# BUTSpeechFIT/VBx

Measured on NVIDIA H100. Metric: x-vectors/sec through 10 VB-HMM EM iters, higher is better.
Workload: dtype f32

## Files before the change

### include/vbx_b200.h

```cpp
#ifndef VBX_B200_H
#define VBX_B200_H

#include <stddef.h>
#include <stdint.h>

#ifdef __cplusplus
extern "C" {
#endif

typedef struct vbx_handle_s *vbx_handle_t;

enum vbx_status {
    VBX_OK = 0,
    VBX_ERR_ARG = -1,
    VBX_ERR_CUDA = -2,
    VBX_ERR_STATE = -3,
    VBX_ERR_NO_DEVICE = -4
};

enum vbx_flag {
    VBX_FLAG_NONFINITE = 1,
    VBX_FLAG_ELBO_DECREASED = 2,
    VBX_FLAG_CONVERGED = 4
};
// ... 134 lines not shown
int vbx_combine_workspace_bytes(vbx_handle_t h, int32_t n_rec, int32_t K, int32_t max_labels, size_t *bytes_out);
int vbx_combine(vbx_handle_t h, int32_t n_rec, const int64_t *offsets, int64_t N, const int64_t *lo, const int64_t *hi,
                int32_t K, const int32_t *labels, const int32_t *labels2, const int32_t *n_labels, int32_t max_labels,
                const double *weights, void *workspace, size_t workspace_bytes, int32_t *labels_out,
                int32_t *labels2_out, int32_t *order_out, double *weights_out, int64_t *D_out, int32_t *map_out,
                int32_t *n_global_out, int32_t *flags_out, int64_t *O_out, int64_t *L_out, void *stream);

int vbx_class_scatter_workspace_bytes(vbx_handle_t h, int64_t N, int32_t D, int32_t K, size_t *bytes_out);
int vbx_class_scatter(vbx_handle_t h, const float *X, int64_t N, int32_t D, int32_t K, const int64_t *offsets,
                      void *workspace, size_t workspace_bytes, double *means_out, double *scatter_out, void *stream);

int vbx_stream_window(vbx_handle_t h, int32_t n, int32_t C, int32_t R, int32_t S_max, int32_t S, const int32_t *slot,
                      const int64_t *blk_off, const int64_t *win_off, const int32_t *blk_lab, const int32_t *n_clusters,
                      const float *blk_fea, double smoothing, const float *ctx_fea, const int32_t *ctx_lab,
                      const int64_t *count, const int32_t *K, const double *n_hist, const double *F_hist, float *fea_out,
                      float *gamma_out, float *pi_out, int32_t *n_states_out, double *prior_n_out, double *prior_F_out,
                      void *stream);
int vbx_stream_commit(vbx_handle_t h, int32_t n, int32_t C, int32_t R, int32_t S_max, const int32_t *slot,
                      const int64_t *blk_off, const int64_t *win_off, const float *blk_fea, const int32_t *first,
                      float *ctx_fea, int32_t *ctx_lab, int64_t *count, int32_t *K, double *n_hist, double *F_hist,
                      int32_t *labels_out, void *stream);

int64_t vbx_launch_count(vbx_handle_t h);

enum vbx_kernel_class {
    VBX_K_PROJECT = 0,
    VBX_K_PREPARE = 1,
    VBX_K_RUN_INIT = 2,
    VBX_K_MSTEP = 3,
    VBX_K_SPEAKER_MODEL = 4,
    VBX_K_LOGLIK = 5,
    VBX_K_FWDBWD = 6,
    VBX_K_EXACT64 = 7,
    VBX_N_KERNEL_CLASSES = 8
};
int vbx_get_timings(vbx_handle_t h, double *ms_out, int64_t *count_out, int32_t reset);

#ifdef __cplusplus
}
#endif
#endif
```

### vbx_b200/_lib.py

```python
import ctypes
import os

_HERE = os.path.dirname(os.path.abspath(__file__))
LIB_PATH = os.environ.get('VBX_B200_LIB', os.path.join(_HERE, 'libvbx_b200.so'))

EXPORTS = ['vbx_version', 'vbx_padded_states', 'vbx_padded_states_wide', 'vbx_create', 'vbx_destroy', 'vbx_last_error',
           'vbx_set_option', 'vbx_plan', 'vbx_bind_workspace', 'vbx_prepare_scale',
           'vbx_prepare_project', 'vbx_prepare_xvectors', 'vbx_run', 'vbx_run_per_recording', 'vbx_hard_labels', 'vbx_hard_labels_keep', 'vbx_ahc_workspace_bytes', 'vbx_ahc', 'vbx_launch_count', 'vbx_get_timings', 'vbx_f64_workspace_bytes',
           'vbx_run_f64', 'vbx_plan_f64', 'vbx_forward_backward', 'vbx_attach_comm', 'vbx_elbo_trace', 'vbx_get_gsum',
           'vbx_score', 'vbx_score_overlap', 'vbx_score_jer', 'vbx_link_batch_workspace_bytes', 'vbx_link_batch',
           'vbx_enroll_batch_workspace_bytes', 'vbx_enroll_batch', 'vbx_cohort_stats_batch_workspace_bytes',
           'vbx_cohort_stats_batch', 'vbx_init_turns', 'vbx_combine_workspace_bytes', 'vbx_combine',
           'vbx_init_random', 'vbx_run_prior', 'vbx_run_f64_prior', 'vbx_class_scatter_workspace_bytes',
           'vbx_class_scatter', 'vbx_stream_window', 'vbx_stream_commit']

FLAG_NONFINITE, FLAG_ELBO_DECREASED, FLAG_CONVERGED = 1, 2, 4
SCORE_BAD_LABEL, SCORE_BAD_REGION, SCORE_BAD_RECORDING = 1, 2, 4
COMBINE_BAD_LABEL, COMBINE_TOO_MANY_LABELS = 1, 2
LINK_MAX_SPEAKERS = 1 << 29
KERNEL_CLASSES = ['project', 'prepare', 'run_init', 'mstep_partial', 'speaker_model', 'loglik', 'forward_backward', 'exact64']


class VbxError(RuntimeError):
    pass


_lib = None


def load():
    global _lib
    if _lib is not None:
        return _lib
    if not os.path.exists(LIB_PATH):
        raise VbxError(f'{LIB_PATH} is missing - run `python -c "import __graft_entry__ as g; g.build()"` '
                       '(there is no CPU fallback for the VB-HMM path)')
    lib = ctypes.CDLL(LIB_PATH)
    vp, i32, i64, dbl = ctypes.c_void_p, ctypes.c_int32, ctypes.c_int64, ctypes.c_double
    lib.vbx_version.restype = ctypes.c_char_p
    lib.vbx_version.argtypes = []
    lib.vbx_padded_states.restype = i32
    lib.vbx_padded_states.argtypes = [i32]
    lib.vbx_padded_states_wide.restype = i32
    lib.vbx_padded_states_wide.argtypes = [i32]
    lib.vbx_create.restype = ctypes.c_int
    lib.vbx_create.argtypes = [i32, ctypes.POINTER(vp)]
    lib.vbx_destroy.restype = ctypes.c_int
    lib.vbx_destroy.argtypes = [vp]
    lib.vbx_last_error.restype = ctypes.c_char_p
    lib.vbx_last_error.argtypes = [vp]
    lib.vbx_set_option.restype = ctypes.c_int
    lib.vbx_set_option.argtypes = [vp, ctypes.c_char_p, i32]
    lib.vbx_plan.restype = ctypes.c_int
# ... 98 lines not shown
```

### vbx_b200/build.py

```python
import os
import subprocess

HERE = os.path.dirname(os.path.abspath(__file__))
CSRC = os.path.join(HERE, 'csrc')
LIB = os.path.join(HERE, 'libvbx_b200.so')
SOURCES = ['vbx_kernels.cu', 'vbx_mma_kernels.cu', 'vbx_long_kernels.cu', 'vbx_fb_split.cu', 'vbx_project_tc.cu', 'vbx_f64.cu', 'vbx_exact64.cu', 'vbx_fb_dense.cu', 'vbx_ahc.cu',
           'vbx_score.cu', 'vbx_count.cu', 'vbx_link.cu', 'vbx_enroll.cu', 'vbx_cohort.cu', 'vbx_init.cu', 'vbx_combine.cu',
           'vbx_train.cu', 'vbx_stream.cu', 'vbx_capi.cu']
ARCH = ['-gencode', 'arch=compute_90a,code=sm_90a']
NVCC_FLAGS = ARCH + ['-lineinfo', '-O3', '-std=c++17', '-Xcompiler', '-fPIC', '-Xptxas', '-v']


def _nvcc():
    for cand in (os.environ.get('NVCC'), '/usr/local/cuda/bin/nvcc', 'nvcc'):
        if cand and (os.path.isabs(cand) and os.path.exists(cand) or not os.path.isabs(cand)):
            return cand
    raise RuntimeError('nvcc not found')


def needs_build():
    if not os.path.exists(LIB):
        return True
    t = os.path.getmtime(LIB)
    deps = [os.path.join(CSRC, f) for f in os.listdir(CSRC) if f.endswith(('.cu', '.cuh', '.h'))]
    deps += [os.path.join(HERE, '..', 'include', 'vbx_b200.h'), os.path.abspath(__file__)]
    return any(os.path.getmtime(d) > t for d in deps)


def build_library(force=False, verbose=False):
    if not force and not needs_build():
        return LIB
    nvcc = _nvcc()
    objs = []
    logs = []
    for src in SOURCES:
        obj = os.path.join(CSRC, src.replace('.cu', '.o'))
        cmd = [nvcc] + NVCC_FLAGS + ['-c', os.path.join(CSRC, src), '-o', obj]
        r = subprocess.run(cmd, capture_output=True, text=True)
        logs.append(r.stderr)
        if r.returncode != 0:
            raise RuntimeError('nvcc failed for %s:\n%s\n%s' % (src, r.stdout, r.stderr))
# ... 15 lines not shown
```

### vbx_b200/csrc/vbx_capi.cu

```cuda
#include <dlfcn.h>
#include <nvtx3/nvToolsExt.h>

#include <algorithm>
#include <cmath>
#include <cstdio>
#include <cstring>
#include <initializer_list>
#include <numeric>
#include <string>
#include <utility>
#include <vector>

#include "../../include/vbx_b200.h"
#include "vbx_internal.cuh"

struct vbx_handle_s {
    int device = 0;
    int sms = 0;
    std::string err;
    vbx::Plan plan;
    vbx::Workspace ws;
    bool planned = false, bound = false, prepared = false;
    bool f64_only = false;
    size_t ws_need = 0;
// ... 348 lines not shown
    if (h->plan_mem) {
        cudaFree(h->plan_mem);
        h->plan_mem = nullptr;
    }
    h->planned = h->bound = h->prepared = false;
    h->f64_only = false;
    drop_graph(h);
    e = cudaMalloc(&h->plan_mem, off);
    if (e != cudaSuccess) return cuda_fail(h, e, "cudaMalloc(plan)");
    char *base = static_cast<char *>(h->plan_mem);
    auto up = [&](size_t o, const void *src, size_t bytes) {
        return bytes ? cudaMemcpy(base + o, src, bytes, cudaMemcpyHostToDevice) : cudaSuccess;
    };
    if ((e = up(o_off, offsets_host, sizeof(int64_t) * (n_rec + 1))) != cudaSuccess ||
        (e = up(o_ord, order.data(), sizeof(int32_t) * n_rec)) != cudaSuccess ||
        (e = up(o_lrec, lrec.data(), sizeof(int32_t) * lrec.size())) != cudaSuccess ||
        (e = up(o_lf0, lf0.data(), sizeof(int64_t) * lf0.size())) != cudaSuccess ||
        (e = up(o_mrec, mrec.data(), sizeof(int32_t) * mrec.size())) != cudaSuccess ||
        (e = up(o_mf0, mf0.data(), sizeof(int64_t) * mf0.size())) != cudaSuccess ||
        (e = up(o_mb, mbegin.data(), sizeof(int32_t) * (n_rec + 1))) != cudaSuccess ||
        (e = up(o_ll, lrec_list.data(), sizeof(int32_t) * lrec_list.size())) != cudaSuccess ||
        (e = up(o_lf, lrec_first.data(), sizeof(int32_t) * lrec_first.size())) != cudaSuccess ||
        (e = up(o_ln, lrec_nchunks.data(), sizeof(int32_t) * lrec_nchunks.size())) != cudaSuccess ||
        (e = up(o_lcr, lchunk_rec.data(), sizeof(int32_t) * lchunk_rec.size())) != cudaSuccess ||
        (e = up(o_lci, lchunk_idx.data(), sizeof(int32_t) * lchunk_idx.size())) != cudaSuccess)
        return cuda_fail(h, e, "cudaMemcpy(plan)");

    vbx::Plan &pl = h->plan;
    pl.n_rec = n_rec;
    pl.R = R;
    pl.S = S;
    pl.exact = h->opt_exact_stop;
    pl.split = split ? 1 : 0;
    pl.n_frames = n_rec ? offsets_host[n_rec] : 0;
    pl.n_ltiles = (int32_t)lrec.size();
    pl.n_mtiles = (int32_t)mrec.size();
    pl.max_T = maxT;
    pl.offsets = reinterpret_cast<const int64_t *>(base + o_off);
    pl.order = reinterpret_cast<const int32_t *>(base + o_ord);
    pl.ltile_rec = reinterpret_cast<const int32_t *>(base + o_lrec);
    pl.ltile_f0 = reinterpret_cast<const int64_t *>(base + o_lf0);
    pl.mtile_rec = reinterpret_cast<const int32_t *>(base + o_mrec);
    pl.mtile_f0 = reinterpret_cast<const int64_t *>(base + o_mf0);
    pl.mtile_begin = reinterpret_cast<const int32_t *>(base + o_mb);
    pl.n_lrec = (int32_t)lrec_list.size();
    pl.n_lchunks = (int32_t)lchunk_rec.size();
    pl.lrec_list = reinterpret_cast<const int32_t *>(base + o_ll);
    pl.lrec_first = reinterpret_cast<const int32_t *>(base + o_lf);
    pl.lrec_nchunks = reinterpret_cast<const int32_t *>(base + o_ln);
    pl.lchunk_rec = reinterpret_cast<const int32_t *>(base + o_lcr);
    pl.lchunk_idx = reinterpret_cast<const int32_t *>(base + o_lci);
    h->ws_need = carve(pl, nullptr, nullptr);
    h->offsets_host.assign(offsets_host, offsets_host + (n_rec ? n_rec + 1 : 0));
    if (n_rec == 0) h->offsets_host.assign(1, 0);
    h->ahc_need = vbx::ahc_workspace_bytes(h->offsets_host.data(), n_rec, &h->ahc_d_off);
    h->planned = true;
    if (workspace_bytes_out) *workspace_bytes_out = h->ws_need;
    return VBX_OK;
}

int vbx_plan_f64(vbx_handle_t h, const int64_t *offsets_host, int32_t n_rec, int32_t R, int32_t S) {
    if (!h || !offsets_host || n_rec < 0) return fail(h, VBX_ERR_ARG, "vbx_plan_f64: null argument");
    if (R < 1 || S < 1 || S > 3600) return fail(h, VBX_ERR_ARG, "vbx_plan_f64: need R >= 1 and 1 <= S <= 3600");
    if (n_rec > 0 && offsets_host[0] != 0) return fail(h, VBX_ERR_ARG, "vbx_plan_f64: offsets[0] must be 0");
    for (int b = 0; b < n_rec; ++b) {
        const int64_t T = offsets_host[b + 1] - offsets_host[b];
// ... 181 lines not shown
    if (!per_rec && !(Fb != 0.0)) return fail(h, VBX_ERR_ARG, w + ": Fb must be non-zero");
    if (per_rec && (!Fa_v || !Fb_v || !loopP_v)) return fail(h, VBX_ERR_ARG, w + ": Fa, Fb and loop_prob must be device arrays [n_rec]");
    if (warm_start && (!alpha_io || !invL_io)) return fail(h, VBX_ERR_ARG, w + ": warm_start needs alpha_io and invL_io");
    const vbx::Plan &pl = h->plan;
    if (pl.n_rec == 0) return VBX_OK;
    if (!Li_out || !n_iters_out || !flags_out || !pi_io) return fail(h, VBX_ERR_ARG, w + ": null output pointer");
    if (pl.n_frames && (!rho || !Phi || !gamma_io)) return fail(h, VBX_ERR_ARG, w + ": null pointer");
    if ((rc = misaligned16(h, w, {{rho, "rho"}, {gamma_io, "gamma_io"}}))) return rc;
    vbx::RunParams rp;
    rp.epsilon = epsilon;
    rp.max_iters = max_iters;
    rp.hybrid = (pl.exact && epsilon > -1e300 && epsilon < 1e300 && max_iters > 1) ? 1 : 0;
    rp.warm = warm_start ? 1 : 0;

    auto enqueue = [&](cudaStream_t st) -> int {
    int rc = 0;
    {
        Timed t(h, st, VBX_K_RUN_INIT);
        rc = counted(h, vbx::launch_run_init(pl, h->ws, gamma_io, n_states, Li_out, n_iters_out, flags_out, max_iters, Fa, Fb,
                                             loop_prob, Fa_v, Fb_v, loopP_v, st), "run_init");
    }
    if (rc) return rc;
    const int rounds = max_iters + (rp.hybrid ? 1 : 0);
    const bool fb_hi = !pl.split && pl.n_rec >= 1024;
    for (int it = 0; it < rounds; ++it) {
        Range nvtx_iter("vbx_em_iteration");
        const bool given = it == 0 && warm_start;
        if (it < max_iters) {
            if (rp.hybrid) {
                Timed t(h, st, VBX_K_EXACT64);
                rc = counted(h, vbx::launch_snapshot(pl, h->ws, gamma_io, pi_io, it, st), "snapshot");
                if (rc) return rc;
            }
            if (!given) {
                Timed t(h, st, VBX_K_MSTEP);
                rc = counted(h, h->opt_gemm ? vbx::launch_mstep_partial(pl, h->ws, rho, gamma_io, st)
                                            : vbx::launch_mstep_mma(pl, h->ws, rho, gamma_io, st), "mstep_partial");
            }
            if (rc) return rc;
            {
                Timed t(h, st, VBX_K_SPEAKER_MODEL);
                rc = counted(h, vbx::launch_speaker_model(pl, h->ws, Phi, n_states, alpha_io, invL_io, given, st, prior_n,
                                                          prior_F), "speaker_model");
            }
            if (rc) return rc;
            {
                Timed t(h, st, VBX_K_LOGLIK);
                rc = counted(h, h->opt_gemm ? vbx::launch_loglik(pl, h->ws, rho, pi_io, n_states, st) : vbx::launch_loglik_mma(pl, h->ws, rho, pi_io, n_states, st), "loglik");
            }
            if (rc) return rc;
            if (fb_hi) {
                cudaEventRecord(h->ev_fork, st);
                cudaStreamWaitEvent(h->hi_stream, h->ev_fork, 0);
            }
            {
                cudaStream_t fs = fb_hi ? h->hi_stream : st;
                Timed t(h, fs, VBX_K_FWDBWD);
                rc = counted(h, vbx::launch_forward_backward(pl, h->ws, rp, gamma_io, pi_io, n_states, Li_out, n_iters_out, flags_out, it, h->opt_fb_spl, h->opt_fb_classic, h->opt_fb_ring, fs), "forward_backward");
            }
            if (fb_hi) {
                cudaEventRecord(h->ev_join, h->hi_stream);
                cudaStreamWaitEvent(st, h->ev_join, 0);
            }
            if (rc) return rc;
        }
        if (rp.hybrid && it > 0) {
            Timed t(h, st, VBX_K_EXACT64);
            rc = counted(h, vbx::launch_exact64_round(pl, h->ws, rp, rho, Phi, gamma_io, pi_io, n_states, alpha_io, invL_io, Li_out,
                                                      n_iters_out, flags_out, st, prior_n, prior_F), "exact64");
            if (rc) return rc;
        }
    }
    return VBX_OK;
    };

    cudaStream_t user = (cudaStream_t)stream;
    const bool want_graph = (h->opt_graph == 1 || (h->opt_graph == 0 && pl.split)) && !h->opt_timing && !h->opt_debug_sync &&
                            !h->graph_broken;
    if (!want_graph) return enqueue(user);
    uint64_t key = 1469598103934665603ull;
    auto mix = [&](uint64_t v) { key = (key ^ v) * 1099511628211ull; };
    auto bits = [](double d) { uint64_t u; memcpy(&u, &d, 8); return u; };
    for (const void *p : {(const void *)rho, (const void *)Phi, (const void *)gamma_io, (const void *)pi_io, (const void *)n_states,
// ... 727 lines not shown
```

### vbx_b200/csrc/vbx_internal.cuh

```cuda
#pragma once
#include <cuda_runtime.h>
#include <stdint.h>

#include <string>
#include <vector>

#define VBX_EPS_TR 1e-8f

namespace vbx {

constexpr int kLTile = 64;
constexpr int kMTile = 512;
constexpr int kLongT = 4096;
constexpr int kChunk = 256;
constexpr int kMaxR = 128;
constexpr int kMaxS = 64;
constexpr int kMaxSWide = 128;
constexpr int kTcMaxD = 2048;

struct Plan {
    int32_t n_rec = 0, R = 0, S = 0;
    int32_t exact = 0;
    int32_t split = 0;
    int64_t n_frames = 0;
    int32_t n_ltiles = 0, n_mtiles = 0;
    int64_t max_T = 0;
    const int64_t *offsets = nullptr;
    const int32_t *order = nullptr;
    const int32_t *ltile_rec = nullptr;
    const int64_t *ltile_f0 = nullptr;
    const int32_t *mtile_rec = nullptr;
    const int64_t *mtile_f0 = nullptr;
    const int32_t *mtile_begin = nullptr;
    int32_t n_lrec = 0, n_lchunks = 0;
    const int32_t *lrec_list = nullptr;
    const int32_t *lrec_first = nullptr;
    const int32_t *lrec_nchunks = nullptr;
    const int32_t *lchunk_rec = nullptr;
    const int32_t *lchunk_idx = nullptr;
};

struct RecParams {
    float Fa, Fb, FaFb, loopP;
    double dFa, dFb, dFaFb, dloopP;
};

struct Workspace {
    float *p = nullptr;
    float *rowmax = nullptr;
    float *rsigma = nullptr;
    float *cvec = nullptr;
    float *partial = nullptr;
    float *A = nullptr;
    float *Afrag_hi = nullptr;
    float *Afrag_lo = nullptr;
    float *bias = nullptr;
// ... 106 lines not shown
    *reinterpret_cast<float4 *>(p) = make_float4(v[0], v[1], v[2], v[3]);
}

__device__ __forceinline__ uint32_t smem_u32(const void *p) { return static_cast<uint32_t>(__cvta_generic_to_shared(p)); }
__device__ __forceinline__ void mbar_init(uint32_t bar, uint32_t count) {
    asm volatile("mbarrier.init.shared::cta.b64 [%0], %1;" ::"r"(bar), "r"(count));
}
__device__ __forceinline__ void mbar_arrive(uint32_t bar) {
    asm volatile("mbarrier.arrive.shared::cta.b64 _, [%0];" ::"r"(bar) : "memory");
}
__device__ __forceinline__ void mbar_expect_tx(uint32_t bar, uint32_t bytes) {
    asm volatile("mbarrier.arrive.expect_tx.shared::cta.b64 _, [%0], %1;" ::"r"(bar), "r"(bytes) : "memory");
}
__device__ __forceinline__ void mbar_add_tx(uint32_t bar, uint32_t bytes) {
    asm volatile("mbarrier.expect_tx.relaxed.cta.shared::cta.b64 [%0], %1;" ::"r"(bar), "r"(bytes) : "memory");
}
__device__ __forceinline__ void mbar_wait(uint32_t bar, uint32_t parity) {
    asm volatile(
        "{\n\t.reg .pred p;\n\t"
        "WAIT_%=:\n\t"
        "mbarrier.try_wait.parity.shared::cta.b64 p, [%0], %1;\n\t"
        "@p bra DONE_%=;\n\t"
        "bra WAIT_%=;\n\t"
        "DONE_%=:\n\t}" ::"r"(bar),
        "r"(parity)
        : "memory");
}
__device__ __forceinline__ void bulk_g2s(uint32_t dst, const void *src, uint32_t bytes, uint32_t bar) {
    asm volatile("cp.async.bulk.shared::cluster.global.mbarrier::complete_tx::bytes [%0], [%1], %2, [%3];" ::"r"(dst),
                 "l"(src), "r"(bytes), "r"(bar)
                 : "memory");
}

__device__ __forceinline__ int find_problem(const int64_t *__restrict__ pref, int G, int64_t x) {
    int lo = 0, hi = G;
    while (hi - lo > 1) {
        const int mid = (lo + hi) >> 1;
        if (pref[mid] <= x) lo = mid;
        else hi = mid;
    }
    return lo;
}

#endif

int launch_prepare_scale(const Plan &pl, const Workspace &ws, const float *fea, const float *Phi, float *rho,
                         cudaStream_t st);
int launch_project_ffma(const Plan &pl, const float *X, int D, const float *V, float *rho, cudaStream_t st);
int launch_g_from_rho(const Plan &pl, const Workspace &ws, const float *rho, const float *Phi, cudaStream_t st);
int launch_run_init(const Plan &pl, const Workspace &ws, const float *gamma, const int32_t *n_states, double *Li,
                    int32_t *n_iters, int32_t *flags, int max_iters, double Fa, double Fb, double loopP,
                    const double *Fa_v, const double *Fb_v, const double *loopP_v, cudaStream_t st);
int launch_mstep_partial(const Plan &pl, const Workspace &ws, const float *rho, const float *gamma, cudaStream_t st);
int launch_speaker_model(const Plan &pl, const Workspace &ws, const float *Phi,
                         const int32_t *n_states, float *alpha_io, float *invL_io, bool from_given,
                         cudaStream_t st, const double *prior_n = nullptr, const double *prior_F = nullptr);
int launch_loglik(const Plan &pl, const Workspace &ws, const float *rho, const float *pi, const int32_t *n_states,
                  cudaStream_t st);
int launch_forward_backward(const Plan &pl, const Workspace &ws, const RunParams &rp, float *gamma, float *pi,
                            const int32_t *n_states, double *Li, int32_t *n_iters, int32_t *flags, int iter,
                            int spl, int classic, int ring, cudaStream_t st);
int launch_elbo_trace(const Plan &pl, const double *Li, int max_iters, double *out, cudaStream_t st);
int launch_forward_backward_split(const Plan &pl, const Workspace &ws, const RunParams &rp, float *gamma, float *pi,
                                  const int32_t *n_states, int spl, cudaStream_t st);
int launch_forward_backward_long(const Plan &pl, const Workspace &ws, const RunParams &rp, float *gamma, float *pi,
                                 const int32_t *n_states, cudaStream_t st);
int launch_mstep_mma(const Plan &pl, const Workspace &ws, const float *rho, const float *gamma, cudaStream_t st);
int launch_loglik_mma(const Plan &pl, const Workspace &ws, const float *rho, const float *pi, const int32_t *n_states,
                      cudaStream_t st);
int launch_snapshot(const Plan &pl, const Workspace &ws, const float *gamma, const float *pi, int iter, cudaStream_t st);
int launch_exact64_round(const Plan &pl, const Workspace &ws, const RunParams &rp, const float *rho, const float *Phi,
                         float *gamma, float *pi, const int32_t *n_states, float *alpha_io, float *invL_io, double *Li,
                         int32_t *n_iters, int32_t *flags, cudaStream_t st, const double *prior_n = nullptr,
                         const double *prior_F = nullptr);
size_t f64_workspace_bytes(const Plan &pl);
int launch_run_f64(const Plan &pl, void *workspace, const double *fea, const double *Phi, double *gamma, double *pi,
                   const int32_t *n_states, double Fa, double Fb, double loopP, int max_iters, double epsilon,
                   double *alpha_io, double *invL_io, int warm, double *Li, int32_t *n_iters, int32_t *flags,
                   cudaStream_t st, const double *prior_n = nullptr, const double *prior_F = nullptr);
int launch_hard_labels(const Plan &pl, const float *gamma, const int32_t *n_states, int32_t *first, int32_t *second,
                       cudaStream_t st);
int launch_hard_labels_keep(const Plan &pl, const float *gamma, const int32_t *n_states, const int32_t *keep,
                            int32_t *first, int32_t *second, double *mass, cudaStream_t st);
int launch_init_turns(const Plan &pl, const int64_t *seg, const int64_t *spk_off, const int64_t *turn_off,
                      const int64_t *turn_lo, const int64_t *turn_hi, const int64_t *turn_cum, const double *smoothing,
                      void *gamma, void *pi, bool f64, cudaStream_t st);
int launch_init_random(const Plan &pl, const uint64_t *rec_key, const uint64_t *seed, const int32_t *n_states,
                       void *gamma, void *pi, bool f64, cudaStream_t st);
int launch_fb_dense(const double *lls, const double *tr, const double *ip, int T, int S, double *post, double *tll,
                    double *lfw, double *lbw, cudaStream_t st);
int launch_score(int n_rec, const int64_t *sys_off, const int64_t *sys_lo, const int64_t *sys_hi, const int64_t *sys_join_hi,
                 const int64_t *reg_off,
                 const int64_t *reg_lo, const int64_t *reg_hi, const uint64_t *reg_mask, const uint8_t *reg_ovl,
                 const int32_t *n_ref, int n_entries, const int32_t *entry_rec, const int64_t *label_off,
                 const int32_t *labels, const int32_t *labels2,
                 const int32_t *n_labels, const int64_t *o_off, int64_t max_cells, int64_t *covered_out,
                 int64_t *fa_out, int64_t *O_out, int32_t *flags_out,
                 const int64_t *t_off, int64_t *T_out,
                 cudaStream_t st);
size_t combine_workspace_bytes(int64_t n_rec, int K, int max_labels);
int launch_combine(int64_t n_rec, const int64_t *offsets, int64_t N, const int64_t *lo, const int64_t *hi, int K,
                   const int32_t *labels, const int32_t *labels2, const int32_t *n_labels_host, int max_labels,
// ... 80 lines not shown
```

### vbx_b200/csrc/vbx_kernels.cu

```cuda
#include <math_constants.h>

#include "vbx_internal.cuh"

namespace vbx {

__device__ __forceinline__ void cp_async16(void *smem, const void *gmem) {
    unsigned s = static_cast<unsigned>(__cvta_generic_to_shared(smem));
    asm volatile("cp.async.cg.shared.global [%0], [%1], 16;\n" ::"r"(s), "l"(gmem));
}
__device__ __forceinline__ void cp_async_wait_all() {
    asm volatile("cp.async.commit_group;\n" ::);
    asm volatile("cp.async.wait_group 0;\n" ::: "memory");
}

template <int LANES>
__device__ __forceinline__ float group_sum(float v) {
#pragma unroll
    for (int off = LANES / 2; off > 0; off >>= 1) v += __shfl_xor_sync(0xffffffffu, v, off);
    return v;
}
template <int LANES>
__device__ __forceinline__ float group_max(float v) {
#pragma unroll
    for (int off = LANES / 2; off > 0; off >>= 1) v = fmaxf(v, __shfl_xor_sync(0xffffffffu, v, off));
    return v;
}
__device__ __forceinline__ double warp_sum_d(double v) {
#pragma unroll
    for (int off = 16; off > 0; off >>= 1) v += __shfl_xor_sync(0xffffffffu, v, off);
    return v;
}

template <int MODE>
__global__ void __launch_bounds__(256) prepare_kernel(Plan pl, Workspace ws, const float *__restrict__ in,
                                                      const float *__restrict__ Phi, float *rho) {
    const int tile = blockIdx.x;
    const int rec = pl.mtile_rec[tile];
    const int64_t f0 = pl.mtile_f0[tile];
    const int len = (int)min((int64_t)kMTile, pl.offsets[rec + 1] - f0);
    const int warp = threadIdx.x >> 5, lane = threadIdx.x & 31;
    const int R = pl.R;
    const bool rlive = 4 * lane < R;
    float4 sc = make_float4(0.f, 0.f, 0.f, 0.f);
    if (rlive) {
        float4 ph = __ldg(reinterpret_cast<const float4 *>(Phi) + lane);
        if (MODE == 0)
            sc = make_float4(sqrtf(ph.x), sqrtf(ph.y), sqrtf(ph.z), sqrtf(ph.w));
        else
            sc = make_float4(1.f / ph.x, 1.f / ph.y, 1.f / ph.z, 1.f / ph.w);
    }
    const double cst = (double)R * 1.8378770664093454835606594728112;
    double gw = 0.0;
    for (int t = warp; t < len; t += 8) {
// ... 1689 lines not shown
```

### vbx_b200/csrc/vbx_mma_kernels.cu

```cuda
#include <math_constants.h>

#include "vbx_internal.cuh"

namespace vbx {

__device__ __forceinline__ void mma_tf32(float (&d)[4], const uint32_t (&a)[4], const uint32_t b0, const uint32_t b1) {
    asm volatile(
        "mma.sync.aligned.m16n8k8.row.col.f32.tf32.tf32.f32 {%0,%1,%2,%3}, {%4,%5,%6,%7}, {%8,%9}, {%0,%1,%2,%3};\n"
        : "+f"(d[0]), "+f"(d[1]), "+f"(d[2]), "+f"(d[3])
        : "r"(a[0]), "r"(a[1]), "r"(a[2]), "r"(a[3]), "r"(b0), "r"(b1));
}
__device__ __forceinline__ void split_tf32(const float x, uint32_t &hi, uint32_t &lo) {
    asm volatile("{\n\t.reg .b32 t;\n\tadd.u32 t, %1, 0x1000;\n\tand.b32 %0, t, 0xffffe000;\n\t}" : "=r"(hi) : "r"(__float_as_uint(x)));
    lo = (__float_as_uint(x - __uint_as_float(hi)) + 0x1000u) & 0xffffe000u;
}
__device__ __forceinline__ void cp_async16_(void *smem, const void *gmem) {
    unsigned s = static_cast<unsigned>(__cvta_generic_to_shared(smem));
    asm volatile("cp.async.cg.shared.global [%0], [%1], 16;\n" ::"r"(s), "l"(gmem));
}

template <int S_PAD>
__global__ void __launch_bounds__(S_PAD > kMaxS ? 256 : 128, S_PAD > kMaxS ? 2 : 4)
    mstep_mma_kernel(Plan pl, Workspace ws, const float *__restrict__ rho, const float *__restrict__ gamma) {
    constexpr int SH = S_PAD > kMaxS ? S_PAD / kMaxS : 1;
    constexpr int SB = S_PAD / SH;
    constexpr int MT = SB > 16 ? SB / 16 : 1;
    constexpr int NTW = 16 / MT;
    constexpr int RW = 8 * NTW;
    constexpr int FS = 4 / MT;
    constexpr int NQ = NTW / 4;
    constexpr int S16 = 16 * MT;
    constexpr int LD = kMaxR + 4;
    __shared__ __align__(16) float red_st[SH > 1 ? 1 : FS][SH > 1 ? 1 : S16][LD];
    extern __shared__ float4 red_dyn[];
    float (*red)[S16 * SH][LD] = SH > 1 ? reinterpret_cast<float (*)[S16 * SH][LD]>(red_dyn) : reinterpret_cast<float (*)[S16 * SH][LD]>(red_st);
    const int tile = blockIdx.x;
    const int rec = pl.mtile_rec[tile];
    if (!ws.active[rec]) return;
    const int64_t f0 = pl.mtile_f0[tile];
    const int len = (int)min((int64_t)kMTile, pl.offsets[rec + 1] - f0);
    const int warp = threadIdx.x >> 5, lane = threadIdx.x & 31;
    const int g = lane >> 2, q = lane & 3;
    const int sh = SH > 1 ? warp >> 2 : 0, w4 = SH > 1 ? (warp & 3) : warp;
    const int rg = w4 % MT, fs = w4 / MT;
    const int R = pl.R;
    const int col0 = rg * RW + 4 * g;
    const float *grow = gamma + f0 * S_PAD + sh * SB;

// ... 367 lines not shown
```

Before: 172.4 million.

## Fuse M-step, speaker model and loglik into one cluster kernel per recording

Adds a thread-block-cluster kernel that, for short recordings (up to two M-tiles, R equal to kMaxR, S in {4,8,16}), runs three steps in one launch. It computes the gamma-weighted rho sums with 3xTF32 MMA, reduces them across the cluster through distributed shared memory, and derives the per-speaker alpha, invL, bias and regularisation terms. It then broadcasts Fa*alpha and the bias to every block with st.async and computes the loglik exponentials from rho still held in shared memory. This replaces three separate launches and their global-memory round trips of partials and rho. The cost is a rigid, specialised code path that needs cluster occupancy checks and falls back when the shape or options don't fit.

```diff
diff --git a/include/vbx_b200.h b/include/vbx_b200.h
--- a/include/vbx_b200.h
+++ b/include/vbx_b200.h
@@ -190,7 +190,8 @@
     VBX_K_LOGLIK = 5,
     VBX_K_FWDBWD = 6,
     VBX_K_EXACT64 = 7,
-    VBX_N_KERNEL_CLASSES = 8
+    VBX_K_EM_CONTRACT = 8,
+    VBX_N_KERNEL_CLASSES = 9
 };
 int vbx_get_timings(vbx_handle_t h, double *ms_out, int64_t *count_out, int32_t reset);
 
diff --git a/vbx_b200/_lib.py b/vbx_b200/_lib.py
--- a/vbx_b200/_lib.py
+++ b/vbx_b200/_lib.py
@@ -18,7 +18,7 @@
 SCORE_BAD_LABEL, SCORE_BAD_REGION, SCORE_BAD_RECORDING = 1, 2, 4
 COMBINE_BAD_LABEL, COMBINE_TOO_MANY_LABELS = 1, 2
 LINK_MAX_SPEAKERS = 1 << 29
-KERNEL_CLASSES = ['project', 'prepare', 'run_init', 'mstep_partial', 'speaker_model', 'loglik', 'forward_backward', 'exact64']
+KERNEL_CLASSES = ['project', 'prepare', 'run_init', 'mstep_partial', 'speaker_model', 'loglik', 'forward_backward', 'exact64', 'em_contract']
 
 
 class VbxError(RuntimeError):
diff --git a/vbx_b200/build.py b/vbx_b200/build.py
--- a/vbx_b200/build.py
+++ b/vbx_b200/build.py
@@ -6,7 +6,7 @@
 LIB = os.path.join(HERE, 'libvbx_b200.so')
 SOURCES = ['vbx_kernels.cu', 'vbx_mma_kernels.cu', 'vbx_long_kernels.cu', 'vbx_fb_split.cu', 'vbx_project_tc.cu', 'vbx_f64.cu', 'vbx_exact64.cu', 'vbx_fb_dense.cu', 'vbx_ahc.cu',
            'vbx_score.cu', 'vbx_count.cu', 'vbx_link.cu', 'vbx_enroll.cu', 'vbx_cohort.cu', 'vbx_init.cu', 'vbx_combine.cu',
-           'vbx_train.cu', 'vbx_stream.cu', 'vbx_capi.cu']
+           'vbx_train.cu', 'vbx_stream.cu', 'vbx_em_contract.cu', 'vbx_capi.cu']
 ARCH = ['-gencode', 'arch=compute_90a,code=sm_90a']
 NVCC_FLAGS = ARCH + ['-lineinfo', '-O3', '-std=c++17', '-Xcompiler', '-fPIC', '-Xptxas', '-v']
 
diff --git a/vbx_b200/csrc/vbx_capi.cu b/vbx_b200/csrc/vbx_capi.cu
--- a/vbx_b200/csrc/vbx_capi.cu
+++ b/vbx_b200/csrc/vbx_capi.cu
@@ -404,6 +404,7 @@
     pl.S = S;
     pl.exact = h->opt_exact_stop;
     pl.split = split ? 1 : 0;
+    pl.em_cluster = vbx::em_contract_cluster(S, R, maxT, split);
     pl.n_frames = n_rec ? offsets_host[n_rec] : 0;
     pl.n_ltiles = (int32_t)lrec.size();
     pl.n_mtiles = (int32_t)mrec.size();
@@ -651,23 +652,30 @@
                 rc = counted(h, vbx::launch_snapshot(pl, h->ws, gamma_io, pi_io, it, st), "snapshot");
                 if (rc) return rc;
             }
-            if (!given) {
-                Timed t(h, st, VBX_K_MSTEP);
-                rc = counted(h, h->opt_gemm ? vbx::launch_mstep_partial(pl, h->ws, rho, gamma_io, st)
-                                            : vbx::launch_mstep_mma(pl, h->ws, rho, gamma_io, st), "mstep_partial");
+            if (pl.em_cluster && !h->opt_gemm && !given && !prior_n) {
+                Timed t(h, st, VBX_K_EM_CONTRACT);
+                rc = counted(h, vbx::launch_em_contract(pl, h->ws, rho, gamma_io, Phi, n_states, alpha_io, invL_io, st),
+                             "em_contract");
+                if (rc) return rc;
+            } else {
+                if (!given) {
+                    Timed t(h, st, VBX_K_MSTEP);
+                    rc = counted(h, h->opt_gemm ? vbx::launch_mstep_partial(pl, h->ws, rho, gamma_io, st)
+                                                : vbx::launch_mstep_mma(pl, h->ws, rho, gamma_io, st), "mstep_partial");
+                }
+                if (rc) return rc;
+                {
+                    Timed t(h, st, VBX_K_SPEAKER_MODEL);
+                    rc = counted(h, vbx::launch_speaker_model(pl, h->ws, Phi, n_states, alpha_io, invL_io, given, st, prior_n,
+                                                              prior_F), "speaker_model");
+                }
+                if (rc) return rc;
+                {
+                    Timed t(h, st, VBX_K_LOGLIK);
+                    rc = counted(h, h->opt_gemm ? vbx::launch_loglik(pl, h->ws, rho, pi_io, n_states, st) : vbx::launch_loglik_mma(pl, h->ws, rho, pi_io, n_states, st), "loglik");
+                }
+                if (rc) return rc;
             }
-            if (rc) return rc;
-            {
-                Timed t(h, st, VBX_K_SPEAKER_MODEL);
-                rc = counted(h, vbx::launch_speaker_model(pl, h->ws, Phi, n_states, alpha_io, invL_io, given, st, prior_n,
-                                                          prior_F), "speaker_model");
-            }
-            if (rc) return rc;
-            {
-                Timed t(h, st, VBX_K_LOGLIK);
-                rc = counted(h, h->opt_gemm ? vbx::launch_loglik(pl, h->ws, rho, pi_io, n_states, st) : vbx::launch_loglik_mma(pl, h->ws, rho, pi_io, n_states, st), "loglik");
-            }
-            if (rc) return rc;
             if (fb_hi) {
                 cudaEventRecord(h->ev_fork, st);
                 cudaStreamWaitEvent(h->hi_stream, h->ev_fork, 0);
diff --git a/vbx_b200/csrc/vbx_em_contract.cu b/vbx_b200/csrc/vbx_em_contract.cu
--- /dev/null
+++ b/vbx_b200/csrc/vbx_em_contract.cu
@@ -0,0 +1,384 @@
+#include <cooperative_groups.h>
+#include <math_constants.h>
+
+#include <mutex>
+
+#include "vbx_internal.cuh"
+
+namespace cg = cooperative_groups;
+
+namespace vbx {
+
+namespace {
+constexpr int kSlots = 4;
+constexpr int kRows = 8;
+constexpr int kHeld = kMTile / kRows / kSlots;
+constexpr int kBars = 4;
+constexpr int kLD = kMaxR + 4;
+constexpr int kRedBytes = 16 * kLD * 4;
+constexpr int kRhoBytes = kHeld * kRows * kMaxR * 4;
+constexpr int kSmemBytes = kRhoBytes + kRedBytes + (kBars + 1) * 8;
+
+__device__ __forceinline__ uint32_t cluster_addr(uint32_t a, uint32_t rank) {
+    uint32_t r;
+    asm volatile("mapa.shared::cluster.u32 %0, %1, %2;" : "=r"(r) : "r"(a), "r"(rank));
+    return r;
+}
+__device__ __forceinline__ void st_async(uint32_t addr, float v, uint32_t bar) {
+    asm volatile("st.async.shared::cluster.mbarrier::complete_tx::bytes.b32 [%0], %1, [%2];" ::"r"(addr),
+                 "r"(__float_as_uint(v)), "r"(bar)
+                 : "memory");
+}
+
+__device__ __forceinline__ float speaker_state(const Workspace &ws, int rec, int S, int s, int r, int ns, float phi, float Fa,
+                                               float FaFb, double gr, float &alpha_out, float &invL_out,
+                                               double (*cpart)[4], double (*rpart)[4]) {
+    const int warp = r >> 5, lane = r & 31;
+    const bool dead = s >= ns;
+    float invL = 1.f, alpha = 0.f, Av = 0.f;
+    float c = 0.f, reg = 0.f;
+    if (!dead) {
+        const float Ns = ws.occ[(int64_t)rec * S + s];
+        invL = 1.f / (1.f + FaFb * Ns * phi);
+        alpha = (float)((double)(FaFb * invL) * gr);
+        Av = Fa * alpha;
+        const float a2 = alpha * alpha;
+        reg = logf(invL) - invL - a2 + 1.f;
+        c = (invL + a2) * phi;
+    }
+    alpha_out = dead ? 0.f : alpha;
+    invL_out = dead ? 0.f : invL;
+    c = group_sum<32>(c);
+    reg = group_sum<32>(reg);
+    if (lane == 0) {
+        cpart[s][warp] = (double)c;
+        rpart[s][warp] = (double)reg;
+    }
+    return Av;
+}
+__device__ __forceinline__ float speaker_bias(const Workspace &ws, int rec, int s, int ns, double (*cpart)[4],
+                                              double (*rpart)[4], double &regp) {
+    const bool dead = s >= ns;
+    regp = dead ? 0.0 : (rpart[s][0] + rpart[s][1]) + (rpart[s][2] + rpart[s][3]);
+    return dead ? CUDART_INF_F : (float)(ws.hp[rec].dFa * 0.5 * ((cpart[s][0] + cpart[s][1]) + (cpart[s][2] + cpart[s][3])));
+}
+}
+
+template <int S_PAD, int CL>
+__global__ void __cluster_dims__(CL, 1, 1) __launch_bounds__(128, 3)
+    em_contract_kernel(Plan pl, Workspace ws, const float *__restrict__ rho, const float *__restrict__ gamma,
+                       const float *__restrict__ Phi, const int32_t *__restrict__ n_states, float *alpha_io,
+                       float *invL_io) {
+    constexpr int S8 = S_PAD > 8 ? S_PAD : 8;
+    constexpr int NT = S8 / 8;
+    constexpr int KS = kMaxR / 8;
+    constexpr int NOWN = (S8 + CL - 1) / CL;
+    static_assert(NT * KS * 64 + S8 <= 16 * kLD && kHeld * kRows * S_PAD <= 16 * kLD, "gamma, Fa*alpha and bias must fit in the slot accumulators' space");
+    extern __shared__ __align__(128) float4 smem4[];
+    float *srho = reinterpret_cast<float *>(smem4);
+    float (*red)[kLD] = reinterpret_cast<float (*)[kLD]>(srho + kHeld * kRows * kMaxR);
+    float *sAv = &red[0][0];
+    float *sbias = sAv + NT * KS * 64;
+    const uint32_t bar0 = smem_u32(srho + kHeld * kRows * kMaxR + 16 * kLD);
+    const uint32_t avbar = bar0 + 8 * kBars;
+    __shared__ double cpart[S8][4], rpart[S8][4];
+
+    cg::cluster_group cluster = cg::this_cluster();
+    const int rank = (int)cluster.block_rank();
+    const int rec = blockIdx.x / CL;
+    if (!ws.active[rec]) return;
+    const int tid = threadIdx.x, warp = tid >> 5, lane = tid & 31;
+    const int g = lane >> 2, q = lane & 3;
+    const int tile = rank / kSlots, fs = rank % kSlots;
+    const int64_t r0 = pl.offsets[rec], T = pl.offsets[rec + 1] - r0;
+    const int ntiles = (int)((T + kMTile - 1) / kMTile);
+    const int64_t f0 = r0 + (int64_t)tile * kMTile;
+    const int len = tile < ntiles ? (int)min((int64_t)kMTile, T - (int64_t)tile * kMTile) : 0;
+    const int nchunks = (len + kRows - 1) / kRows;
+    const int nmine = nchunks > fs ? (nchunks - fs + kSlots - 1) / kSlots : 0;
+    const int nmt = (nmine + 1) >> 1;
+
+    if (tid == 0) {
+        for (int b = 0; b <= kBars; ++b) mbar_init(bar0 + 8 * b, 1);
+        asm volatile("fence.mbarrier_init.release.cluster;" ::: "memory");
+        mbar_expect_tx(avbar, (NT * KS * 64 + S_PAD) * 4);
+    }
+    __syncthreads();
+    auto chunk_rows = [&](int i) { return min(kRows, len - kRows * (fs + kSlots * i)); };
+    float *sgam = &red[0][0];
+    if (warp == 0) {
+        if (lane < kBars && kHeld / kBars * lane < nmine) {
+            uint32_t bytes = 0;
+            for (int i = kHeld / kBars * lane; i < min(nmine, kHeld / kBars * (lane + 1)); ++i)
+                bytes += chunk_rows(i) * (kMaxR + S_PAD) * 4;
+            mbar_expect_tx(bar0 + 8 * lane, bytes);
+        }
+        __syncwarp();
+        if (lane < nmine) {
+            const int64_t fr = f0 + kRows * (fs + kSlots * lane);
+            const uint32_t bar = bar0 + 8 * (lane / (kHeld / kBars));
+            bulk_g2s(smem_u32(srho + lane * kRows * kMaxR), rho + fr * kMaxR, chunk_rows(lane) * kMaxR * 4, bar);
+            bulk_g2s(smem_u32(sgam + lane * kRows * S_PAD), gamma + fr * S_PAD, chunk_rows(lane) * S_PAD * 4, bar);
+        }
+    }
+    {
+        const int valid = nmine ? kRows * (nmine - 1) + chunk_rows(nmine - 1) : 0;
+        float4 *z = reinterpret_cast<float4 *>(srho);
+        for (int i = valid * (kMaxR / 4) + tid; i < 2 * nmt * kRows * (kMaxR / 4); i += 128) z[i] = make_float4(0.f, 0.f, 0.f, 0.f);
+    }
+    __syncthreads();
+
+    {
+        float acc[4][4];
+#pragma unroll
+        for (int e = 0; e < 4; ++e) acc[e][0] = acc[e][1] = acc[e][2] = acc[e][3] = 0.f;
+        const int s0c = min(g, S_PAD - 1), s1c = min(g + 8, S_PAD - 1);
+        const bool v0 = g < S_PAD, v1 = g + 8 < S_PAD;
+        for (int i = 0; i < nmine; ++i) {
+            const int c = fs + kSlots * i;
+            const bool va = 8 * c + q < len, vb = 8 * c + q + 4 < len;
+            if (i % (kHeld / kBars) == 0) mbar_wait(bar0 + 8 * (i / (kHeld / kBars)), 0);
+            const float *ga = sgam + (i * kRows + q) * S_PAD, *gb = ga + 4 * S_PAD;
+            uint32_t ah[4], al[4];
+            split_tf32((va && v0) ? ga[s0c] : 0.f, ah[0], al[0]);
+            split_tf32((va && v1) ? ga[s1c] : 0.f, ah[1], al[1]);
+            split_tf32((vb && v0) ? gb[s0c] : 0.f, ah[2], al[2]);
+            split_tf32((vb && v1) ? gb[s1c] : 0.f, ah[3], al[3]);
+            const float4 x0 = *reinterpret_cast<const float4 *>(srho + (i * kRows + q) * kMaxR + 32 * warp + 4 * g);
+            const float4 x1 = *reinterpret_cast<const float4 *>(srho + (i * kRows + q + 4) * kMaxR + 32 * warp + 4 * g);
+            const float b0v[4] = {x0.x, x0.y, x0.z, x0.w};
+            const float b1v[4] = {x1.x, x1.y, x1.z, x1.w};
+#pragma unroll
+            for (int e = 0; e < 4; ++e) {
+                uint32_t bh0, bl0, bh1, bl1;
+                split_tf32(b0v[e], bh0, bl0);
+                split_tf32(b1v[e], bh1, bl1);
+                mma_tf32(acc[e], al, bh0, bh1);
+                mma_tf32(acc[e], ah, bl0, bl1);
+                mma_tf32(acc[e], ah, bh0, bh1);
+            }
+        }
+        __syncthreads();
+#pragma unroll
+        for (int e = 0; e < 4; ++e) {
+            const int c0 = 32 * warp + 8 * q + e, c1 = c0 + 4;
+            red[g][c0] = acc[e][0];
+            red[g][c1] = acc[e][1];
+            red[g + 8][c0] = acc[e][2];
+            red[g + 8][c1] = acc[e][3];
+        }
+    }
+    cluster.sync();
+
+    const int ns = n_states ? n_states[rec] : S_PAD;
+    float avs[NOWN], alphas[NOWN], invLs[NOWN];
+    {
+        const float phi = Phi[tid];
+        const float Fa = ws.hp[rec].Fa, FaFb = ws.hp[rec].FaFb;
+#pragma unroll
+        for (int k = 0; k < NOWN; ++k) {
+            const int s = rank + CL * k;
+            avs[k] = 0.f;
+            if (s < S8) {
+                double gr = 0.0;
+                if (s < ns)
+                    for (int t = 0; t < ntiles; ++t) {
+                        float v = cluster.map_shared_rank(&red[s][tid], kSlots * t)[0];
+#pragma unroll
+                        for (int k2 = 1; k2 < kSlots; ++k2) v += cluster.map_shared_rank(&red[s][tid], kSlots * t + k2)[0];
+                        gr += (double)v;
+                    }
+                avs[k] = speaker_state(ws, rec, S_PAD, s, tid, ns, phi, Fa, FaFb, gr, alphas[k], invLs[k], cpart, rpart);
+            }
+        }
+    }
+    __syncthreads();
+    float own_bias = 0.f;
+    double own_regp = 0.0;
+    if (tid < NOWN && rank + CL * tid < S_PAD) own_bias = speaker_bias(ws, rec, rank + CL * tid, ns, cpart, rpart, own_regp);
+    cluster.sync();
+    {
+        const int r = tid, j = 2 * (r >> 4) + ((r >> 1) & 1), fq = (r >> 2) & 3, e = r & 1;
+#pragma unroll
+        for (int k = 0; k < NOWN; ++k) {
+            const int s = rank + CL * k;
+            if (s < S8) {
+                const uint32_t a = smem_u32(sAv + (((s >> 3) * KS + j) * 32 + 4 * (s & 7) + fq) * 2 + e);
+#pragma unroll
+                for (int p = 0; p < CL; ++p) st_async(cluster_addr(a, p), avs[k], cluster_addr(avbar, p));
+            }
+        }
+        if (tid < NOWN && rank + CL * tid < S_PAD) {
+            const int s = rank + CL * tid;
+#pragma unroll
+            for (int p = 0; p < CL; ++p) st_async(cluster_addr(smem_u32(sbias + s), p), own_bias, cluster_addr(avbar, p));
+            ws.bias[(int64_t)rec * S_PAD + s] = own_bias;
+            ws.regp[(int64_t)rec * S_PAD + s] = own_regp;
+        }
+#pragma unroll
+        for (int k = 0; k < NOWN; ++k) {
+            const int s = rank + CL * k;
+            if (s < S_PAD) {
+                const int64_t o = ((int64_t)rec * S_PAD + s) * kMaxR + tid;
+                if (alpha_io) alpha_io[o] = alphas[k];
+                if (invL_io) invL_io[o] = invLs[k];
+            }
+        }
+    }
+    mbar_wait(avbar, 0);
+
+    float nb[NT][2];
+#pragma unroll
+    for (int i = 0; i < NT; ++i) {
+        const int s = 8 * i + 2 * q;
+        nb[i][0] = s < S_PAD ? -sbias[s] : -CUDART_INF_F;
+        nb[i][1] = s + 1 < S_PAD ? -sbias[s + 1] : -CUDART_INF_F;
+    }
+    const uint2 *sB = reinterpret_cast<const uint2 *>(sAv);
+    if (warp < nmt) {
+        float D[2][NT][4], E[2][NT][4];
+#pragma unroll
+        for (int m = 0; m < 2; ++m)
+#pragma unroll
+            for (int i = 0; i < NT; ++i) {
+                D[m][i][0] = nb[i][0];
+                D[m][i][1] = nb[i][1];
+                D[m][i][2] = nb[i][0];
+                D[m][i][3] = nb[i][1];
+                E[m][i][0] = E[m][i][1] = E[m][i][2] = E[m][i][3] = 0.f;
+            }
+        const float4 *pa[2], *pb[2];
+#pragma unroll
+        for (int m = 0; m < 2; ++m) {
+            pa[m] = reinterpret_cast<const float4 *>(srho + (16 * (warp + 4 * m) + 2 * g) * kMaxR + 4 * q);
+            pb[m] = reinterpret_cast<const float4 *>(srho + (16 * (warp + 4 * m) + 2 * g + 1) * kMaxR + 4 * q);
+        }
+#pragma unroll
+        for (int k = 0; k < 8; ++k) {
+            float4 xa[2], xb[2];
+#pragma unroll
+            for (int m = 0; m < 2; ++m) {
+                xa[m] = pa[m][4 * k];
+                xb[m] = pb[m][4 * k];
+            }
+#pragma unroll
+            for (int h = 0; h < 2; ++h) {
+                const int j = 2 * k + h;
+                uint32_t ah[2][4], al[2][4];
+#pragma unroll
+                for (int m = 0; m < 2; ++m) {
+                    split_tf32(h ? xa[m].z : xa[m].x, ah[m][0], al[m][0]);
+                    split_tf32(h ? xb[m].z : xb[m].x, ah[m][1], al[m][1]);
+                    split_tf32(h ? xa[m].w : xa[m].y, ah[m][2], al[m][2]);
+                    split_tf32(h ? xb[m].w : xb[m].y, ah[m][3], al[m][3]);
+                }
+#pragma unroll
+                for (int i = 0; i < NT; ++i) {
+                    const uint2 b = sB[(i * KS + j) * 32 + lane];
+                    const uint32_t hx = b.x & 0xffffe000u, hy = b.y & 0xffffe000u;
+                    const uint32_t lx = __float_as_uint(__uint_as_float(b.x) - __uint_as_float(hx));
+                    const uint32_t ly = __float_as_uint(__uint_as_float(b.y) - __uint_as_float(hy));
+#pragma unroll
+                    for (int m = 0; m < 2; ++m) {
+                        mma_tf32(E[m][i], al[m], hx, hy);
+                        mma_tf32(D[m][i], ah[m], hx, hy);
+                        mma_tf32(E[m][i], ah[m], lx, ly);
+                    }
+                }
+            }
+        }
+#pragma unroll
+        for (int m = 0; m < 2; ++m) {
+#pragma unroll
+            for (int i = 0; i < NT; ++i)
+#pragma unroll
+                for (int e = 0; e < 4; ++e) D[m][i][e] += E[m][i][e];
+            float m0 = fmaxf(D[m][0][0], D[m][0][1]), m1 = fmaxf(D[m][0][2], D[m][0][3]);
+#pragma unroll
+            for (int i = 1; i < NT; ++i) {
+                m0 = fmaxf(m0, fmaxf(D[m][i][0], D[m][i][1]));
+                m1 = fmaxf(m1, fmaxf(D[m][i][2], D[m][i][3]));
+            }
+            m0 = fmaxf(m0, __shfl_xor_sync(0xffffffffu, m0, 1));
+            m1 = fmaxf(m1, __shfl_xor_sync(0xffffffffu, m1, 1));
+            m0 = fmaxf(m0, __shfl_xor_sync(0xffffffffu, m0, 2));
+            m1 = fmaxf(m1, __shfl_xor_sync(0xffffffffu, m1, 2));
+            const int u = warp + 4 * m;
+            const int ta = kRows * (fs + kSlots * (2 * u + (g >> 2))) + 2 * (g & 3), tb = ta + 1;
+#pragma unroll
+            for (int i = 0; i < NT; ++i) {
+                const int s = 8 * i + 2 * q;
+                if (s < S_PAD) {
+                    const float2 va = make_float2(expf(D[m][i][0] - m0), expf(D[m][i][1] - m0));
+                    const float2 vb = make_float2(expf(D[m][i][2] - m1), expf(D[m][i][3] - m1));
+                    if (ta < len) *reinterpret_cast<float2 *>(ws.p + (f0 + ta) * S_PAD + s) = va;
+                    if (tb < len) *reinterpret_cast<float2 *>(ws.p + (f0 + tb) * S_PAD + s) = vb;
+                }
+            }
+            if (q == 0) {
+                if (ta < len) ws.rowmax[f0 + ta] = m0;
+                if (tb < len) ws.rowmax[f0 + tb] = m1;
+            }
+        }
+    }
+}
+
+template <int S_PAD, int CL>
+static int em_contract_cluster_t() {
+    constexpr int kMaxDevices = 64;
+    static std::mutex mu;
+    static int ok[kMaxDevices];
+    static bool init = false;
+    int dev = 0;
+    if (cudaGetDevice(&dev) != cudaSuccess || dev < 0 || dev >= kMaxDevices) return (void)cudaGetLastError(), 0;
+    std::lock_guard<std::mutex> lock(mu);
+    if (!init) {
+        for (int &v : ok) v = -1;
+        init = true;
+    }
+    if (ok[dev] < 0) {
+        ok[dev] = 0;
+        if (cudaFuncSetAttribute(em_contract_kernel<S_PAD, CL>, cudaFuncAttributeMaxDynamicSharedMemorySize, kSmemBytes) != cudaSuccess)
+            return (void)cudaGetLastError(), 0;
+        cudaLaunchConfig_t cfg = {};
+        cfg.gridDim = dim3(CL);
+        cfg.blockDim = dim3(128);
+        cfg.dynamicSmemBytes = kSmemBytes;
+        int n = 0;
+        if (cudaOccupancyMaxActiveClusters(&n, em_contract_kernel<S_PAD, CL>, &cfg) != cudaSuccess) return (void)cudaGetLastError(), 0;
+        ok[dev] = n >= 1;
+    }
+    return ok[dev] ? CL : 0;
+}
+
+int em_contract_cluster(int S, int R, int64_t max_T, bool split) {
+    if (split || R != kMaxR || max_T > 2 * kMTile) return 0;
+    const bool two = max_T > kMTile;
+    switch (S) {
+        case 4: return two ? em_contract_cluster_t<4, 8>() : em_contract_cluster_t<4, 4>();
+        case 8: return two ? em_contract_cluster_t<8, 8>() : em_contract_cluster_t<8, 4>();
+        case 16: return two ? em_contract_cluster_t<16, 8>() : em_contract_cluster_t<16, 4>();
+        default: return 0;
+    }
+}
+
+int launch_em_contract(const Plan &pl, const Workspace &ws, const float *rho, const float *gamma, const float *Phi,
+                       const int32_t *n_states, float *alpha_io, float *invL_io, cudaStream_t st) {
+    if (pl.n_rec == 0) return 0;
+    const int CL = pl.em_cluster;
+#define VBX_EMC(S_, CL_)                                                                                                 \
+    em_contract_kernel<S_, CL_><<<pl.n_rec * CL_, 128, kSmemBytes, st>>>(pl, ws, rho, gamma, Phi, n_states, alpha_io, invL_io)
+    switch (pl.S * 16 + CL) {
+        case 4 * 16 + 4: VBX_EMC(4, 4); break;
+        case 4 * 16 + 8: VBX_EMC(4, 8); break;
+        case 8 * 16 + 4: VBX_EMC(8, 4); break;
+        case 8 * 16 + 8: VBX_EMC(8, 8); break;
+        case 16 * 16 + 4: VBX_EMC(16, 4); break;
+        case 16 * 16 + 8: VBX_EMC(16, 8); break;
+        default: return -1;
+    }
+#undef VBX_EMC
+    return cudaGetLastError() == cudaSuccess ? 1 : -1;
+}
+
+}
diff --git a/vbx_b200/csrc/vbx_internal.cuh b/vbx_b200/csrc/vbx_internal.cuh
--- a/vbx_b200/csrc/vbx_internal.cuh
+++ b/vbx_b200/csrc/vbx_internal.cuh
@@ -22,6 +22,7 @@
     int32_t n_rec = 0, R = 0, S = 0;
     int32_t exact = 0;
     int32_t split = 0;
+    int32_t em_cluster = 0;
     int64_t n_frames = 0;
     int32_t n_ltiles = 0, n_mtiles = 0;
     int64_t max_T = 0;
@@ -194,6 +195,23 @@
                  : "memory");
 }
 
+__device__ __forceinline__ void mma_tf32(float (&d)[4], const uint32_t (&a)[4], const uint32_t b0, const uint32_t b1) {
+    asm volatile(
+        "mma.sync.aligned.m16n8k8.row.col.f32.tf32.tf32.f32 {%0,%1,%2,%3}, {%4,%5,%6,%7}, {%8,%9}, {%0,%1,%2,%3};\n"
+        : "+f"(d[0]), "+f"(d[1]), "+f"(d[2]), "+f"(d[3])
+        : "r"(a[0]), "r"(a[1]), "r"(a[2]), "r"(a[3]), "r"(b0), "r"(b1));
+}
+__device__ __forceinline__ void split_tf32(const float x, uint32_t &hi, uint32_t &lo) {
+    asm volatile("{\n\t.reg .b32 t;\n\tadd.u32 t, %1, 0x1000;\n\tand.b32 %0, t, 0xffffe000;\n\t}" : "=r"(hi) : "r"(__float_as_uint(x)));
+    lo = (__float_as_uint(x - __uint_as_float(hi)) + 0x1000u) & 0xffffe000u;
+}
+template <int LANES>
+__device__ __forceinline__ float group_sum(float v) {
+#pragma unroll
+    for (int off = LANES / 2; off > 0; off >>= 1) v += __shfl_xor_sync(0xffffffffu, v, off);
+    return v;
+}
+
 __device__ __forceinline__ int find_problem(const int64_t *__restrict__ pref, int G, int64_t x) {
     int lo = 0, hi = G;
     while (hi - lo > 1) {
@@ -230,6 +248,9 @@
 int launch_mstep_mma(const Plan &pl, const Workspace &ws, const float *rho, const float *gamma, cudaStream_t st);
 int launch_loglik_mma(const Plan &pl, const Workspace &ws, const float *rho, const float *pi, const int32_t *n_states,
                       cudaStream_t st);
+int em_contract_cluster(int S, int R, int64_t max_T, bool split);
+int launch_em_contract(const Plan &pl, const Workspace &ws, const float *rho, const float *gamma, const float *Phi,
+                       const int32_t *n_states, float *alpha_io, float *invL_io, cudaStream_t st);
 int launch_snapshot(const Plan &pl, const Workspace &ws, const float *gamma, const float *pi, int iter, cudaStream_t st);
 int launch_exact64_round(const Plan &pl, const Workspace &ws, const RunParams &rp, const float *rho, const float *Phi,
                          float *gamma, float *pi, const int32_t *n_states, float *alpha_io, float *invL_io, double *Li,
diff --git a/vbx_b200/csrc/vbx_kernels.cu b/vbx_b200/csrc/vbx_kernels.cu
--- a/vbx_b200/csrc/vbx_kernels.cu
+++ b/vbx_b200/csrc/vbx_kernels.cu
@@ -13,12 +13,6 @@
     asm volatile("cp.async.wait_group 0;\n" ::: "memory");
 }
 
-template <int LANES>
-__device__ __forceinline__ float group_sum(float v) {
-#pragma unroll
-    for (int off = LANES / 2; off > 0; off >>= 1) v += __shfl_xor_sync(0xffffffffu, v, off);
-    return v;
-}
 template <int LANES>
 __device__ __forceinline__ float group_max(float v) {
 #pragma unroll
diff --git a/vbx_b200/csrc/vbx_mma_kernels.cu b/vbx_b200/csrc/vbx_mma_kernels.cu
--- a/vbx_b200/csrc/vbx_mma_kernels.cu
+++ b/vbx_b200/csrc/vbx_mma_kernels.cu
@@ -4,16 +4,6 @@
 
 namespace vbx {
 
-__device__ __forceinline__ void mma_tf32(float (&d)[4], const uint32_t (&a)[4], const uint32_t b0, const uint32_t b1) {
-    asm volatile(
-        "mma.sync.aligned.m16n8k8.row.col.f32.tf32.tf32.f32 {%0,%1,%2,%3}, {%4,%5,%6,%7}, {%8,%9}, {%0,%1,%2,%3};\n"
-        : "+f"(d[0]), "+f"(d[1]), "+f"(d[2]), "+f"(d[3])
-        : "r"(a[0]), "r"(a[1]), "r"(a[2]), "r"(a[3]), "r"(b0), "r"(b1));
-}
-__device__ __forceinline__ void split_tf32(const float x, uint32_t &hi, uint32_t &lo) {
-    asm volatile("{\n\t.reg .b32 t;\n\tadd.u32 t, %1, 0x1000;\n\tand.b32 %0, t, 0xffffe000;\n\t}" : "=r"(hi) : "r"(__float_as_uint(x)));
-    lo = (__float_as_uint(x - __uint_as_float(hi)) + 0x1000u) & 0xffffe000u;
-}
 __device__ __forceinline__ void cp_async16_(void *smem, const void *gmem) {
     unsigned s = static_cast<unsigned>(__cvta_generic_to_shared(smem));
     asm volatile("cp.async.cg.shared.global [%0], [%1], 16;\n" ::"r"(s), "l"(gmem));
```

Result: faster. 194.7 million (median of 6 runs) (+12.9%).
